# khanhha/temporal_inverse_kinematics

Hardware: AMD Instinct MI355X
Metric: IK frames/sec (COCO-17->SMPLx pose) (higher is better)
Workload: dtype f32 via bf16x3 (x = 3 bf16 planes, 6 MFMA products, fp32 accumulate; fp32 exponent range); 1 GPU; ST-GCN IK forward, batch=1024x64-frame x COCO-17 windows per GPU -> (B,4,66) SMPL-X pose; global_batch=1024, window_frames=64, out_frames=4, parallelism=single

## Files before the change

### temporal_inverse_kinematics_amd/csrc/debug.cpp

```cpp
#include <hip/hip_runtime.h>

#include <algorithm>
#include <map>
#include <mutex>

#include "misc.h"
#include "model.h"

namespace tik_host {
std::atomic<int> g_alloc_fill{-1};
thread_local Profiler* g_prof = nullptr;

bool guard_mode() {
    static const bool on = getenv("TIK_GUARD") && getenv("TIK_GUARD")[0] == '1';
    return on;
}
static std::mutex g_guard_mu;
static std::map<void*, size_t> g_guard_bufs;
void guard_register(void* base, size_t bytes) {
    std::lock_guard<std::mutex> l(g_guard_mu);
    g_guard_bufs[base] = bytes;
}
void guard_unregister(void* base) {
    std::lock_guard<std::mutex> l(g_guard_mu);
    g_guard_bufs.erase(base);
}

static bool checksum_mode() {
    static const bool on = getenv("TIK_CHECKSUM") != nullptr;
    return on;
}
static std::string g_cks;
static unsigned long long* g_cks_dev = nullptr;

ProfScope::~ProfScope() {
    if (g_prof) g_prof->end(i, st);
    if (checksum_mode() && op) {
        if (!g_cks_dev) (void)hipMalloc(&g_cks_dev, 8);
        unsigned long long h = 0;
        (void)hipMemsetAsync(g_cks_dev, 0, 8, st);
        (void)tik::launch_checksum(op, obytes, g_cks_dev, st);
        (void)hipMemcpyAsync(&h, g_cks_dev, 8, hipMemcpyDeviceToHost, st);
        (void)hipStreamSynchronize(st);
        char b[160];
        snprintf(b, sizeof(b), "%s:%llx;", lab, h);
        g_cks += b;
    }
}

template <class Launch, class Report>
static hipError_t launch_traced(size_t slots, hipStream_t st, Launch launch, Report report) {
    static const bool on = getenv("TIK_X_TRACE") != nullptr;
    if (!on) return launch(nullptr);
    unsigned long long* d = nullptr;
    hipError_t e = hipMalloc(&d, slots * 8);
    if (e != hipSuccess) return e;
    (void)hipMemset(d, 0, slots * 8);
    e = launch(d);
    if (e == hipSuccess) e = hipStreamSynchronize(st);
    std::vector<unsigned long long> h(slots);
    if (e == hipSuccess) e = hipMemcpy(h.data(), d, slots * 8, hipMemcpyDeviceToHost);
    (void)hipFree(d);
    report(h);
    return e;
}

hipError_t launch_xgemm_traced(tik::XArgs a, int bn, int epi, hipStream_t st, const char* label) {
    const int rt = tik::xgemm_tile_rows(epi);
    const long long nwg = (long long)((a.M + rt - 1) / rt) * ((a.Nc + bn - 1) / bn);
    return launch_traced(nwg * 8, st,
        [&](unsigned long long* d) { a.trace = d; return tik::launch_xgemm(a, bn, epi, st); },
        [&](const std::vector<unsigned long long>& h) {
            double s[5] = {0, 0, 0, 0, 0}, n = 0, ks = 0;
            for (long long w = 0; w < nwg; ++w) {
                if (!h[8 * w + 6]) continue;
                n += 1; ks = (double)h[8 * w + 5];
                for (int k = 0; k < 5; ++k) s[k] += (double)h[8 * w + k];
            }
            n = std::max(1.0, n);
            fprintf(stderr, "XTRACE %-10s wg %6.0f ksteps %3.0f | cycles/wg: prologue %7.0f main %8.0f epi %7.0f | "
                    "barrier %7.0f vmwait %7.0f | main/kstep %6.0f\n", label, n, ks, s[0] / n, s[1] / n, s[2] / n,
                    s[3] / n, s[4] / n, s[1] / n / std::max(1.0, ks));
        });
}

hipError_t launch_xgraph_traced(tik::XGraphArgs a, int ncu, hipStream_t st, const char* label) {
    return launch_traced((size_t)ncu * 16, st,
        [&](unsigned long long* d) { a.trace = d; return tik::launch_xgraph(a, ncu, st); },
        [&](const std::vector<unsigned long long>& h) {
            double s0[8] = {0}, s4[8] = {0}, n = 0;
            for (int w = 0; w < ncu; ++w) {
                if (!h[16 * w + 6]) continue;
                n += 1;
                for (int k = 0; k < 8; ++k) { s0[k] += (double)h[16 * w + k]; s4[k] += (double)h[16 * w + 8 + k]; }
            }
            const double ns = std::max(1.0, s0[6]);
            fprintf(stderr, "XGTRACE %-8s wgs %4.0f steps/wg %5.1f total/wg %8.0f | per step, wave0: bar %6.0f mfma0-3 %6.0f split %6.0f load %6.0f mfma4-16 %6.0f epi %6.0f"
                    " | wave4: bar %6.0f mfma0-3 %6.0f split %6.0f load %6.0f mfma4-16 %6.0f epi %6.0f\n", label, n, s0[6] / std::max(1.0, n),
                    s0[7] / std::max(1.0, n), s0[0] / ns, s0[1] / ns, s0[2] / ns, s0[3] / ns, s0[4] / ns, s0[5] / ns, s4[0] / ns, s4[1] / ns,
                    s4[2] / ns, s4[3] / ns, s4[4] / ns, s4[5] / ns);
        });
}

hipError_t launch_xblock_traced(tik::XBlkArgs a, bool raw, int ncu, hipStream_t st, const char* label) {
    return launch_traced((size_t)ncu * 24, st,
        [&](unsigned long long* d) { a.trace = d; return tik::launch_xblock(a, raw, ncu, st); },
        [&](const std::vector<unsigned long long>& h) {
            double s0[8] = {0}, s4[8] = {0}, nt = 0;
            for (int w = 0; w < ncu; ++w) {
                if (!h[24 * w + 9]) continue;
                nt += (double)h[24 * w + 8];
                for (int k = 0; k < 8; ++k) { s0[k] += (double)h[24 * w + k]; s4[k] += (double)h[24 * w + 12 + k]; }
            }
            nt = std::max(1.0, nt);
            fprintf(stderr, "XBTRACE %-8s tiles %6.0f | per tile, wave0: start %6.0f G+mix %6.0f zbar %6.0f res %6.0f bar+dma %6.0f T %6.0f endbar %6.0f"
                    " | wave4: start %6.0f G+mix %6.0f zbar %6.0f res %6.0f bar+dma %6.0f T %6.0f endbar %6.0f\n", label, nt,
                    s0[0] / nt, s0[1] / nt, s0[2] / nt, (s0[3] + s0[6]) / nt, s0[7] / nt, s0[4] / nt, s0[5] / nt, s4[0] / nt, s4[1] / nt,
                    s4[2] / nt, (s4[3] + s4[6]) / nt, s4[7] / nt, s4[4] / nt, s4[5] / nt);
        });
}

}
using namespace tik_host;

extern "C" {

int tik_debug_checksums(char* buf, int len) {
    if (!checksum_mode()) return fail(TIK_E_INVALID, "TIK_CHECKSUM is not set");
    const int n = (int)g_cks.size();
    if (buf && len > 0) {
        strncpy(buf, g_cks.c_str(), len - 1);
        buf[len - 1] = 0;
    }
    g_cks.clear();
    return n;
}

int tik_debug_check_guards(void) {
    if (!guard_mode()) return fail(TIK_E_INVALID, "TIK_GUARD=1 is not set");
    HIP_TRY(hipDeviceSynchronize());
    std::lock_guard<std::mutex> l(g_guard_mu);
    std::vector<unsigned char> h(GUARD_BYTES);
    int bad = 0;
    std::string rep;
    for (const auto& kv : g_guard_bufs) {
        const char* base = static_cast<const char*>(kv.first);
        for (int side = 0; side < 2; ++side) {
            const char* gp = side == 0 ? base : base + GUARD_BYTES + kv.second;
            HIP_TRY(hipMemcpy(h.data(), gp, GUARD_BYTES, hipMemcpyDeviceToHost));
            size_t first = GUARD_BYTES, last = 0, cnt = 0;
            bool clean = true;
            for (size_t i = 0; i < GUARD_BYTES && clean; i += 8) {
                unsigned long long w;
                memcpy(&w, h.data() + i, 8);
                clean = w == 0xA5A5A5A5A5A5A5A5ull;
            }
            for (size_t i = 0; i < GUARD_BYTES && !clean; ++i)
                if (h[i] != 0xA5) { first = std::min(first, i); last = i; ++cnt; }
            if (cnt) {
                ++bad;
                char b[256];
                snprintf(b, sizeof(b), "[buf %p payload %zu B: %s guard, %zu bytes changed at +%zu..+%zu] ", (const void*)(base + GUARD_BYTES),
                         kv.second, side == 0 ? "front" : "back", cnt, first, last);
                rep += b;
                HIP_TRY(hipMemset(const_cast<char*>(gp), 0xA5, GUARD_BYTES));
            }
        }
    }
    g_err = rep;
    return bad;
}

int tik_debug_alloc_fill(void) { return g_alloc_fill.load(); }

}
```

### temporal_inverse_kinematics_amd/csrc/xgraph.h

```cpp
#pragma once
#include <hip/hip_runtime.h>

namespace tik {

struct XGraphArgs {
    int nframes;
    const float* x;
    int ldx;
    int cin, cout;
    const unsigned short* wp;
    const float* bias2;
    const float* amix;
    int mix_sparse;
    float* out;
    int ldo;
    int nts;
    float* trash;
    int tune;
    unsigned long long* trace;
};

bool xgraph_ok(const XGraphArgs& a);
hipError_t launch_xgraph(const XGraphArgs& a, int ncu, hipStream_t st);

}
```

### temporal_inverse_kinematics_amd/csrc/xgraph.hip

```cpp
#include <algorithm>
#include <type_traits>

#include "xgemm_dev.h"
#include "xgraph.h"

namespace tik {

namespace xg {
constexpr int V = 17, FR = 16, PX = FR * V;
constexpr int NU = PX * 8;
constexpr int NLD = (NU + 511) / 512;
constexpr int PROWB = 3 * 32 * 2;
constexpr int PBYTES = PX * PROWB;
}

__device__ __forceinline__ int xg_unit(int R, int p, int u) { return R * xg::PROWB + ((p * 4 + (u ^ ((R >> 1) & 3))) << 4); }

__device__ f32x4 tik_llvm_raw_buffer_load_v4f32(i32x4 rsrc, int voffset, int soffset, int aux)
    __asm("llvm.amdgcn.raw.buffer.load.v4f32");

typedef __bf16 xbf16x4 __attribute__((ext_vector_type(4)));

#ifdef TIK_XTUNE
#define XG_OFF(bit) (a.tune & (bit))
#else
#define XG_OFF(bit) false
#endif

template <int NK, int NP>
__global__ __launch_bounds__(512, 1) void xgraph_kernel(XGraphArgs a) {
    using namespace xg;
    constexpr int D = NK <= 4 ? 2 : 1;
    constexpr int B2MAX = V * 256 * 4;
    __shared__ __attribute__((aligned(16))) unsigned char smem[2 * PBYTES + B2MAX];
    float* const b2s = reinterpret_cast<float*>(smem + 2 * PBYTES);
    auto pimg = [&](int s) __attribute__((always_inline)) { return smem + (s & 1) * PBYTES; };

    int tid = threadIdx.x, lane = tid & 63;
    const int wave = __builtin_amdgcn_readfirstlane(tid >> 6);
    const int QO = a.nframes, M = QO * V;
    constexpr int npass = NP;
    const int nfg = (QO + FR - 1) / FR;
    const int ntiles = nfg * npass;
    int t_begin, t_end;
    {
        const int nwg = gridDim.x, s = xcd_slot(blockIdx.x, nwg);
        t_begin = (int)((long long)s * ntiles / nwg);
        t_end = (int)((long long)(s + 1) * ntiles / nwg);
    }
    if (t_begin >= t_end) return;
    const int total = (t_end - t_begin) * NK;
    auto tile_fg = [&](int t) __attribute__((always_inline)) { return t / npass; };
    auto tile_pass = [&](int t) __attribute__((always_inline)) { return t - (t / npass) * npass; };

    for (int i = tid; i < V * a.cout; i += 512) b2s[i] = a.bias2[i];
    float amv[5];
#pragma unroll
    for (int k = 0; k < 5; ++k) amv[k] = 64 * k + lane < V * V ? a.amix[64 * k + lane] : 0.f;

    const i32x4 rX = buf_rsrc(a.x, (unsigned)((long long)M * a.ldx * 4));
    f32x4 rb[D][NLD];
    auto load_unit = [&](int s, f32x4 (&r)[NLD], int i) __attribute__((always_inline)) {
        const int t = t_begin + s / NK, kb = s - (s / NK) * NK;
        const int q0 = tile_fg(t) * FR;
        const bool live = s < total;
        const int U = 512 * i + tid, m = U >> 3, u = U & 7;
        const int q = q0 + m / V;
        const unsigned off = live && U < NU && q < QO && !XG_OFF(1) ? (unsigned)(((long long)q0 * V + m) * a.ldx * 4 + kb * 128 + u * 16) : DMA_OOB;
        r[i] = tik_llvm_raw_buffer_load_v4f32(rX, (int)off, 0, 2);
    };
    auto load = [&](int s, f32x4 (&r)[NLD]) __attribute__((always_inline)) {
#pragma unroll
        for (int i = 0; i < NLD; ++i) load_unit(s, r, i);
    };
    auto split_unit = [&](int s, const f32x4 (&r)[NLD], int i) __attribute__((always_inline)) {
        unsigned char* P = pimg(s);
        const int U = 512 * i + tid;
        if (i + 1 < NLD || U < NU) {
            const int m = U >> 3, u = U & 7;
            const int R = 16 * (m % V) + m / V;
            xbf16x4 p0, p1, p2;
#pragma unroll
            for (int e = 0; e < 4; ++e) {
                const float x = r[i][e];
                const __bf16 b0 = (__bf16)x;
                const float r1 = x - (float)b0;
                const __bf16 b1 = (__bf16)r1;
                p0[e] = b0;
                p1[e] = b1;
                p2[e] = (__bf16)(r1 - (float)b1);
            }
            const int h = (u & 1) * 8;
            *reinterpret_cast<xbf16x4*>(P + xg_unit(R, 0, u >> 1) + h) = p0;
            *reinterpret_cast<xbf16x4*>(P + xg_unit(R, 1, u >> 1) + h) = p1;
            *reinterpret_cast<xbf16x4*>(P + xg_unit(R, 2, u >> 1) + h) = p2;
        }
    };
    auto split = [&](int s, const f32x4 (&r)[NLD]) __attribute__((always_inline)) {
#pragma unroll
        for (int i = 0; i < NLD; ++i) split_unit(s, r, i);
    };

    xbf16x8 w[NK][3];
    auto load_wk = [&](int pass, int kb) __attribute__((always_inline)) {
        const int cg = pass * 8 + wave;
#pragma unroll
        for (int p = 0; p < 3; ++p)
            w[kb][p] = *reinterpret_cast<const xbf16x8*>(a.wp + ((((size_t)cg * NK + kb) * 3 + p) * 64 + lane) * 8);
    };
    auto load_w = [&](int pass) __attribute__((always_inline)) {
#pragma unroll
        for (int kb = 0; kb < NK; ++kb) load_wk(pass, kb);
    };

    load(0, rb[0]);
    load_w(tile_pass(t_begin));
    split(0, rb[0]);
#pragma unroll
    for (int d = 1; d <= D; ++d) load(d, rb[d % D]);

    f32x4 acc[V];
#pragma unroll
    for (int j = 0; j < V; ++j) acc[j] = f32x4{0.f, 0.f, 0.f, 0.f};

#ifdef TIK_XTRACE
    const bool tr = a.trace != nullptr && (wave == 0 || wave == 4);
#else
    constexpr bool tr = false;
#endif
    unsigned long long ph_[6] = {0, 0, 0, 0, 0, 0}, tlast = 0, tstart = 0;
    auto stamp = [&](int i) __attribute__((always_inline)) {
        if (tr) {
            const unsigned long long t = __builtin_amdgcn_s_memtime();
            if (i >= 0) ph_[i] += t - tlast;
            else tstart = t;
            tlast = t;
        }
    };
    stamp(-1);

    auto step = [&](int s, int t, int pass, auto KBc) __attribute__((always_inline)) {
        constexpr int kb = decltype(KBc)::value;
        constexpr int nb = (kb + 1) % D;
        asm volatile("" : "+v"(tid), "+v"(lane));
        const int g = lane >> 4, f = lane & 15;
        lds_barrier();
        stamp(0);
        const unsigned char* P = pimg(s);
        constexpr int XPF = 2;
        xbf16x8 xb[XPF + 1][3];
        auto rd = [&](int j, xbf16x8 (&d)[3]) __attribute__((always_inline)) {
#pragma unroll
            for (int p = 0; p < 3; ++p) d[p] = *reinterpret_cast<const xbf16x8*>(P + xg_unit(16 * j + f, p, g));
        };
        auto mfma_j = [&](int j) __attribute__((always_inline)) {
            if (j + XPF < V) rd(j + XPF, xb[(j + XPF) % (XPF + 1)]);
            __builtin_amdgcn_sched_barrier(0);
            if (XG_OFF(4)) return;
            const xbf16x8(&x)[3] = xb[j % (XPF + 1)];
            acc[j] = __builtin_amdgcn_mfma_f32_16x16x32_bf16(w[kb][0], x[2], acc[j], 0, 0, 0);
            acc[j] = __builtin_amdgcn_mfma_f32_16x16x32_bf16(w[kb][1], x[1], acc[j], 0, 0, 0);
            acc[j] = __builtin_amdgcn_mfma_f32_16x16x32_bf16(w[kb][2], x[0], acc[j], 0, 0, 0);
            acc[j] = __builtin_amdgcn_mfma_f32_16x16x32_bf16(w[kb][0], x[1], acc[j], 0, 0, 0);
            acc[j] = __builtin_amdgcn_mfma_f32_16x16x32_bf16(w[kb][1], x[0], acc[j], 0, 0, 0);
            acc[j] = __builtin_amdgcn_mfma_f32_16x16x32_bf16(w[kb][0], x[0], acc[j], 0, 0, 0);
            __builtin_amdgcn_sched_barrier(0);
        };
#pragma unroll
        for (int j = 0; j < XPF; ++j) rd(j, xb[j]);
        if constexpr (NP == 2) {
#pragma unroll
            for (int j = 0; j < V; ++j) {
                mfma_j(j);
                if (j % 3 == 1 && j / 3 < NLD) {
                    const int i = j / 3;
                    if (!XG_OFF(2)) split_unit(s + 1, rb[nb], i);
                    load_unit(s + 1 + D, rb[nb], i);
                    asm volatile("" ::: "memory");
                    __builtin_amdgcn_sched_barrier(0);
                }
                if (j == 3) {
                    stamp(1);
                    stamp(2);
                    stamp(3);
                }
            }
        } else {
#pragma unroll
            for (int j = 0; j < 4; ++j) mfma_j(j);
            stamp(1);
            if (!XG_OFF(2)) split(s + 1, rb[nb]);
            stamp(2);
            load(s + 1 + D, rb[nb]);
            stamp(3);
#pragma unroll
            for (int j = 4; j < V; ++j) mfma_j(j);
        }
        stamp(4);
        if constexpr (NP == 2) load_wk(tile_pass(t + 1), kb);
        if constexpr (kb == NK - 1) {
            const int co = pass * 128 + 16 * wave + 4 * g;
            const int q = tile_fg(t) * FR + f;
            auto mix_all = [&](auto sparse) __attribute__((always_inline)) {
                constexpr bool SP = decltype(sparse)::value;
#pragma unroll
                for (int wj = 0; wj < V; ++wj) {
                    f32x4 z = *reinterpret_cast<const f32x4*>(b2s + wj * a.cout + co);
#pragma unroll
                    for (int v = 0; v < V; ++v)
                        if (XG_OFF(16)) {
                            if (v == wj) z += acc[v];
                        } else if (!SP || ((coco_hop2_mask3(wj) >> v) & 1u)) {
                            const float av = __builtin_bit_cast(
                                float, __builtin_amdgcn_readlane(__builtin_bit_cast(int, amv[(v * V + wj) / 64]), (v * V + wj) % 64));
                            z += av * acc[v];
                        }
#pragma unroll
                    for (int e = 0; e < 4; ++e) z[e] = z[e] > 0.f ? z[e] : 0.f;
                    float* o = q < QO ? a.out + ((size_t)q * V + wj) * a.ldo + co : a.trash;
                    if (!XG_OFF(8)) xst4(o, z, a.nts);
                }
            };
            if (a.mix_sparse) mix_all(std::true_type{});
            else mix_all(std::false_type{});
#pragma unroll
            for (int j = 0; j < V; ++j) acc[j] = f32x4{0.f, 0.f, 0.f, 0.f};
            stamp(5);
        }
    };
    for (int t = t_begin; t < t_end; ++t) {
        const int s0 = (t - t_begin) * NK, pass = tile_pass(t);
        step(s0, t, pass, std::integral_constant<int, 0>{});
        step(s0 + 1, t, pass, std::integral_constant<int, 1>{});
        if constexpr (NK > 2) {
            step(s0 + 2, t, pass, std::integral_constant<int, 2>{});
            step(s0 + 3, t, pass, std::integral_constant<int, 3>{});
        }
        if constexpr (NK > 4) {
            step(s0 + 4, t, pass, std::integral_constant<int, 4>{});
            step(s0 + 5, t, pass, std::integral_constant<int, 5>{});
            step(s0 + 6, t, pass, std::integral_constant<int, 6>{});
            step(s0 + 7, t, pass, std::integral_constant<int, 7>{});
        }
    }
    asm volatile("s_waitcnt vmcnt(0)" ::: "memory");
#ifdef TIK_XTRACE
    if (tr && lane == 0) {
        unsigned long long* o = a.trace + 16 * (size_t)blockIdx.x + (wave == 4 ? 8 : 0);
#pragma unroll
        for (int i = 0; i < 6; ++i) o[i] = ph_[i];
        o[6] = (unsigned long long)total;
        o[7] = tlast - tstart;
    }
#endif
}

bool xgraph_ok(const XGraphArgs& a) {
    return (a.cin == 64 || a.cin == 128 || a.cin == 256) && (a.cout == 128 || a.cout == 256) && a.ldx % 4 == 0 &&
           a.ldx >= a.cin && a.ldo % 4 == 0 && a.ldo >= a.cout;
}

hipError_t launch_xgraph(const XGraphArgs& a, int ncu, hipStream_t st) {
    if (a.nframes <= 0) return hipSuccess;
    if (!xgraph_ok(a) || !a.x || !a.wp || !a.bias2 || !a.amix || !a.out || !a.trash || ncu <= 0) return hipErrorInvalidValue;
    const long long row_bytes = 17LL * a.ldx * 4;
    const int chunk = (int)std::min<long long>(a.nframes, ((1LL << 31) - 1) / row_bytes / xg::FR * xg::FR);
    if (chunk <= 0) return hipErrorInvalidValue;
    (void)hipGetLastError();
    for (int q0 = 0; q0 < a.nframes; q0 += chunk) {
        XGraphArgs c = a;
        c.nframes = std::min(chunk, a.nframes - q0);
        c.x = a.x + (size_t)q0 * 17 * a.ldx;
        c.out = a.out + (size_t)q0 * 17 * a.ldo;
        const int ntiles = ((c.nframes + xg::FR - 1) / xg::FR) * (a.cout / 128);
        const int grid = std::min(ntiles, ncu);
        const bool two = a.cout == 256;
        if (a.cin == 64) hipLaunchKernelGGL((two ? xgraph_kernel<2, 2> : xgraph_kernel<2, 1>), dim3(grid), dim3(512), 0, st, c);
        else if (a.cin == 128) hipLaunchKernelGGL((two ? xgraph_kernel<4, 2> : xgraph_kernel<4, 1>), dim3(grid), dim3(512), 0, st, c);
        else hipLaunchKernelGGL((two ? xgraph_kernel<8, 2> : xgraph_kernel<8, 1>), dim3(grid), dim3(512), 0, st, c);
        const hipError_t e = hipGetLastError();
        if (e != hipSuccess) return e;
    }
    return hipSuccess;
}

}
```

Measured before the change: 351,200 IK frames/s.

## Pin each xgraph workgroup to one output-channel pass to keep weights resident

Changes the persistent xgraph kernel's work split. Each workgroup now owns a single output-channel pass and a contiguous range of frame groups, instead of interleaving tiles across both passes. Weights are loaded once per workgroup rather than reloaded for the next tile's pass inside every k-step. This removes per-step weight traffic for the cout=256 case. The cost is that the same input frames are read by two workgroups, one per pass, and load balance changes when the CU count is not divisible by the pass count.

```diff
diff --git a/temporal_inverse_kinematics_amd/csrc/debug.cpp b/temporal_inverse_kinematics_amd/csrc/debug.cpp
--- a/temporal_inverse_kinematics_amd/csrc/debug.cpp
+++ b/temporal_inverse_kinematics_amd/csrc/debug.cpp
@@ -85,11 +85,12 @@
 }
 
 hipError_t launch_xgraph_traced(tik::XGraphArgs a, int ncu, hipStream_t st, const char* label) {
-    return launch_traced((size_t)ncu * 16, st,
+    const int nwg = std::max(ncu, 2);
+    return launch_traced((size_t)nwg * 16, st,
         [&](unsigned long long* d) { a.trace = d; return tik::launch_xgraph(a, ncu, st); },
         [&](const std::vector<unsigned long long>& h) {
             double s0[8] = {0}, s4[8] = {0}, n = 0;
-            for (int w = 0; w < ncu; ++w) {
+            for (int w = 0; w < nwg; ++w) {
                 if (!h[16 * w + 6]) continue;
                 n += 1;
                 for (int k = 0; k < 8; ++k) { s0[k] += (double)h[16 * w + k]; s4[k] += (double)h[16 * w + 8 + k]; }
diff --git a/temporal_inverse_kinematics_amd/csrc/xgraph.h b/temporal_inverse_kinematics_amd/csrc/xgraph.h
--- a/temporal_inverse_kinematics_amd/csrc/xgraph.h
+++ b/temporal_inverse_kinematics_amd/csrc/xgraph.h
@@ -20,6 +20,19 @@
     unsigned long long* trace;
 };
 
+struct XGraphRun {
+    int pass, fg_begin, fg_end;
+};
+__host__ __device__ inline XGraphRun xgraph_run(int slot, int grid, int nfg, int npass) {
+    const int nset = grid / npass, i = slot / npass;
+    if (i >= nset) return {0, 0, 0};
+    return {slot - i * npass, (int)((long long)i * nfg / nset), (int)((long long)(i + 1) * nfg / nset)};
+}
+inline int xgraph_grid(int nfg, int ncu, int npass) {
+    const int nset = ncu / npass > 1 ? ncu / npass : 1;
+    return (nfg < nset ? nfg : nset) * npass;
+}
+
 bool xgraph_ok(const XGraphArgs& a);
 hipError_t launch_xgraph(const XGraphArgs& a, int ncu, hipStream_t st);
 
diff --git a/temporal_inverse_kinematics_amd/csrc/xgraph.hip b/temporal_inverse_kinematics_amd/csrc/xgraph.hip
--- a/temporal_inverse_kinematics_amd/csrc/xgraph.hip
+++ b/temporal_inverse_kinematics_amd/csrc/xgraph.hip
@@ -39,19 +39,10 @@
     int tid = threadIdx.x, lane = tid & 63;
     const int wave = __builtin_amdgcn_readfirstlane(tid >> 6);
     const int QO = a.nframes, M = QO * V;
-    constexpr int npass = NP;
-    const int nfg = (QO + FR - 1) / FR;
-    const int ntiles = nfg * npass;
-    int t_begin, t_end;
-    {
-        const int nwg = gridDim.x, s = xcd_slot(blockIdx.x, nwg);
-        t_begin = (int)((long long)s * ntiles / nwg);
-        t_end = (int)((long long)(s + 1) * ntiles / nwg);
-    }
+    const XGraphRun run = xgraph_run(xcd_slot(blockIdx.x, gridDim.x), gridDim.x, (QO + FR - 1) / FR, NP);
+    const int pass = run.pass, t_begin = run.fg_begin, t_end = run.fg_end;
     if (t_begin >= t_end) return;
     const int total = (t_end - t_begin) * NK;
-    auto tile_fg = [&](int t) __attribute__((always_inline)) { return t / npass; };
-    auto tile_pass = [&](int t) __attribute__((always_inline)) { return t - (t / npass) * npass; };
 
     for (int i = tid; i < V * a.cout; i += 512) b2s[i] = a.bias2[i];
     float amv[5];
@@ -62,7 +53,7 @@
     f32x4 rb[D][NLD];
     auto load_unit = [&](int s, f32x4 (&r)[NLD], int i) __attribute__((always_inline)) {
         const int t = t_begin + s / NK, kb = s - (s / NK) * NK;
-        const int q0 = tile_fg(t) * FR;
+        const int q0 = t * FR;
         const bool live = s < total;
         const int U = 512 * i + tid, m = U >> 3, u = U & 7;
         const int q = q0 + m / V;
@@ -102,19 +93,17 @@
     };
 
     xbf16x8 w[NK][3];
-    auto load_wk = [&](int pass, int kb) __attribute__((always_inline)) {
+    auto load_w = [&]() __attribute__((always_inline)) {
         const int cg = pass * 8 + wave;
 #pragma unroll
-        for (int p = 0; p < 3; ++p)
-            w[kb][p] = *reinterpret_cast<const xbf16x8*>(a.wp + ((((size_t)cg * NK + kb) * 3 + p) * 64 + lane) * 8);
-    };
-    auto load_w = [&](int pass) __attribute__((always_inline)) {
-#pragma unroll
-        for (int kb = 0; kb < NK; ++kb) load_wk(pass, kb);
+        for (int kb = 0; kb < NK; ++kb)
+#pragma unroll
+            for (int p = 0; p < 3; ++p)
+                w[kb][p] = *reinterpret_cast<const xbf16x8*>(a.wp + ((((size_t)cg * NK + kb) * 3 + p) * 64 + lane) * 8);
     };
 
     load(0, rb[0]);
-    load_w(tile_pass(t_begin));
+    load_w();
     split(0, rb[0]);
 #pragma unroll
     for (int d = 1; d <= D; ++d) load(d, rb[d % D]);
@@ -139,7 +128,7 @@
     };
     stamp(-1);
 
-    auto step = [&](int s, int t, int pass, auto KBc) __attribute__((always_inline)) {
+    auto step = [&](int s, int t, auto KBc) __attribute__((always_inline)) {
         constexpr int kb = decltype(KBc)::value;
         constexpr int nb = (kb + 1) % D;
         asm volatile("" : "+v"(tid), "+v"(lane));
@@ -197,10 +186,9 @@
             for (int j = 4; j < V; ++j) mfma_j(j);
         }
         stamp(4);
-        if constexpr (NP == 2) load_wk(tile_pass(t + 1), kb);
         if constexpr (kb == NK - 1) {
             const int co = pass * 128 + 16 * wave + 4 * g;
-            const int q = tile_fg(t) * FR + f;
+            const int q = t * FR + f;
             auto mix_all = [&](auto sparse) __attribute__((always_inline)) {
                 constexpr bool SP = decltype(sparse)::value;
 #pragma unroll
@@ -229,18 +217,18 @@
         }
     };
     for (int t = t_begin; t < t_end; ++t) {
-        const int s0 = (t - t_begin) * NK, pass = tile_pass(t);
-        step(s0, t, pass, std::integral_constant<int, 0>{});
-        step(s0 + 1, t, pass, std::integral_constant<int, 1>{});
+        const int s0 = (t - t_begin) * NK;
+        step(s0, t, std::integral_constant<int, 0>{});
+        step(s0 + 1, t, std::integral_constant<int, 1>{});
         if constexpr (NK > 2) {
-            step(s0 + 2, t, pass, std::integral_constant<int, 2>{});
-            step(s0 + 3, t, pass, std::integral_constant<int, 3>{});
+            step(s0 + 2, t, std::integral_constant<int, 2>{});
+            step(s0 + 3, t, std::integral_constant<int, 3>{});
         }
         if constexpr (NK > 4) {
-            step(s0 + 4, t, pass, std::integral_constant<int, 4>{});
-            step(s0 + 5, t, pass, std::integral_constant<int, 5>{});
-            step(s0 + 6, t, pass, std::integral_constant<int, 6>{});
-            step(s0 + 7, t, pass, std::integral_constant<int, 7>{});
+            step(s0 + 4, t, std::integral_constant<int, 4>{});
+            step(s0 + 5, t, std::integral_constant<int, 5>{});
+            step(s0 + 6, t, std::integral_constant<int, 6>{});
+            step(s0 + 7, t, std::integral_constant<int, 7>{});
         }
     }
     asm volatile("s_waitcnt vmcnt(0)" ::: "memory");
@@ -272,9 +260,8 @@
         c.nframes = std::min(chunk, a.nframes - q0);
         c.x = a.x + (size_t)q0 * 17 * a.ldx;
         c.out = a.out + (size_t)q0 * 17 * a.ldo;
-        const int ntiles = ((c.nframes + xg::FR - 1) / xg::FR) * (a.cout / 128);
-        const int grid = std::min(ntiles, ncu);
         const bool two = a.cout == 256;
+        const int grid = xgraph_grid((c.nframes + xg::FR - 1) / xg::FR, ncu, two ? 2 : 1);
         if (a.cin == 64) hipLaunchKernelGGL((two ? xgraph_kernel<2, 2> : xgraph_kernel<2, 1>), dim3(grid), dim3(512), 0, st, c);
         else if (a.cin == 128) hipLaunchKernelGGL((two ? xgraph_kernel<4, 2> : xgraph_kernel<4, 1>), dim3(grid), dim3(512), 0, st, c);
         else hipLaunchKernelGGL((two ? xgraph_kernel<8, 2> : xgraph_kernel<8, 1>), dim3(grid), dim3(512), 0, st, c);
```

After: 352,300 IK frames/s, median of 6. Within noise of the previous version (+0.3%).
